# pkuyzy/ESC-GNN

Measured on AMD Instinct MI355X. Metric: graphs/sec + edges-aggregated/sec, NestedGIN_eff h=3 bs=128 @1/2/4/8 GPU, higher is better.
Workload: dtype f32; 1 GPU; count_cycle-shaped random regular graphs (n in 10/15/20/30), target=triangles, NestedGIN_eff h=3 layers=4 hidden=256, bs=128 per GPU (configs[1]); global_batch=128, parallelism=dp1 graph-sharded, rccl_ranks=1, ranks=1

## Files before the change

esc-gnn_amd/_native.py:

```python
import ctypes
import os
from ctypes import c_double, c_int64

from . import _abi

_HERE = os.path.dirname(os.path.abspath(__file__))
LIB_PATH = os.path.join(_HERE, "libescgnn_hip.so")


class NativeLibraryError(ImportError):
    pass


try:
    _ABI = _abi.load()
except OSError as exc:
    raise NativeLibraryError("esc_gnn_amd: cannot read the C header %s the binding is derived from (%s)" % (_abi.HEADER, exc)) from exc


def const(name):
    return _ABI.constants[name]


def struct(name):
# ... 45 lines not shown
LAPPE_SIGNATURES = {name: args for name, (args, _) in _LAPPE.functions.items()}
_RET.update({name: ret for name, (_, ret) in _LAPPE.functions.items()})
RWSE_HEADER = os.path.join(os.path.dirname(_abi.HEADER), "escgnn_rwse.h")
try:
    _RWSE = _abi.load(RWSE_HEADER)
except OSError as exc:
    raise NativeLibraryError("esc_gnn_amd: cannot read the C header %s the binding is derived from (%s)" % (RWSE_HEADER, exc)) from exc
RWSE_SIGNATURES = {name: args for name, (args, _) in _RWSE.functions.items()}
_RET.update({name: ret for name, (_, ret) in _RWSE.functions.items()})
STEP_HEADER = os.path.join(os.path.dirname(_abi.HEADER), "escgnn_step.h")
try:
    _STEP = _abi.load(STEP_HEADER)
except OSError as exc:
    raise NativeLibraryError("esc_gnn_amd: cannot read the C header %s the binding is derived from (%s)" % (STEP_HEADER, exc)) from exc
STEP_SIGNATURES = {name: args for name, (args, _) in _STEP.functions.items()}
_RET.update({name: ret for name, (_, ret) in _STEP.functions.items()})
GATEDGCN_HEADER = os.path.join(os.path.dirname(_abi.HEADER), "escgnn_gatedgcn.h")
try:
    _GATED = _abi.load(GATEDGCN_HEADER)
except OSError as exc:
    raise NativeLibraryError("esc_gnn_amd: cannot read the C header %s the binding is derived from (%s)" % (GATEDGCN_HEADER, exc)) from exc
GATEDGCN_SIGNATURES = {name: args for name, (args, _) in _GATED.functions.items()}
_RET.update({name: ret for name, (_, ret) in _GATED.functions.items()})
KIND = {name[len("ESC_K_"):].lower(): v for name, v in _ABI.enum.items() if name != "ESC_K_COUNT"}

CollateArgs = struct("esc_collate_args")
BnFuse = struct("esc_bn_fuse")
BnFold = struct("esc_bn_fold")
BnBwdFused = struct("esc_bn_bwd_fused")
BnBwdNext = struct("esc_bn_bwd_next")
SumJob = struct("esc_sum_job")
ReduceJob = struct("esc_reduce_job")

_lib = None


def lib():
    global _lib
    if _lib is not None:
        return _lib
    if not os.path.exists(LIB_PATH):
        raise NativeLibraryError(
            "esc_gnn_amd: %s not found. The HIP hot path has no fallback — build it with "
            "`python -c 'import __graft_entry__ as g; g.build()'` or `make -C esc-gnn_amd/csrc`." % LIB_PATH)
    h = ctypes.CDLL(LIB_PATH)
    for name, args in list(SIGNATURES.items()) + list(EXTENSION_SIGNATURES.items()) + list(I2GNN_SIGNATURES.items()) + list(GINEPLUS_SIGNATURES.items()) + list(GPS_SIGNATURES.items()) + list(LAPPE_SIGNATURES.items()) + list(RWSE_SIGNATURES.items()) + list(STEP_SIGNATURES.items()) + list(GATEDGCN_SIGNATURES.items()):
        try:
            fn = getattr(h, name)
        except AttributeError as exc:
            raise NativeLibraryError("esc_gnn_amd: %s lacks symbol %s (stale build?)" % (LIB_PATH, name)) from exc
        fn.argtypes = args
        fn.restype = _RET[name]
    if h.esc_abi_version() != ABI_VERSION:
        raise NativeLibraryError("esc_gnn_amd: ABI version mismatch (library %d, header %d) — rebuild"
                                 % (h.esc_abi_version(), ABI_VERSION))
    _lib = h
    return h


def call(name, *args):
    h = lib()
    rc = getattr(h, name)(*args)
    if rc != 0:
        raise RuntimeError("%s failed (%d): %s" % (name, rc, h.esc_last_error().decode()))


def ptr(t):
    return None if t is None else t.data_ptr()

# ... 35 lines not shown
```

esc-gnn_amd/csrc/engine.hip:

```cpp
#include "common.h"
#include "../../include/escgnn_step.h"

#include <map>
#include <vector>
#include <cstdlib>

namespace esc {

struct Arena {
  float* base;
  int64_t off;
  float* take(int64_t n) {
    float* p = base ? base + off : nullptr;
    off += (n + 63) & ~63LL;
    return p;
  }
};

struct BnWs { float *mean, *invstd, *scale, *shift, *nglob, *coef; };
struct MlpWs { float *Y0, *Y1; BnWs b0, b1; float* A1 = nullptr; };

struct Layout {
  int64_t N, E, Z, H, L, C0, W;
  float *Zb, *Yz; BnWs zb0, zb1;
// ... 117 lines not shown
  return esc_linear_bwd_both_deferred(dY, ld_dy, X, ld_x, sc, sh, lin.w, K, M, N, K, dX, ld_dx, accumulate, lin.dw, K, lin.db,
                                      slabs, &c.jobs->back(), c.s);
}

static constexpr bool kBnBwdApplyInGemm = true;
static constexpr bool kBnBwdSumsFromDx = true;
static constexpr bool kBnBwdSumsFromAgg = true;
static esc_bn_bwd_fused bn_fused(const float* x, int64_t ld_x, const BnWs& w, int relu) {
  return esc_bn_bwd_fused{x, ld_x, w.mean, w.invstd, w.scale, w.shift, w.coef, relu};
}
static int linear_backward_bn(const Ctx& c, const float* dOut, int64_t ld_dout, const esc_bn_bwd_fused& f, const float* X, int64_t ld_x,
                              const float* sc, const float* sh, const esc_linear_t& lin, int64_t M, float* dX, int64_t ld_dx,
                              int accumulate, const esc_bn_bwd_next* next) {
  const LdsFloorGuard cap(c.on_edge_stream);
  const int64_t N = lin.out_dim, K = lin.in_dim;
  if (c.jobs == nullptr)
    return esc_linear_bwd_both_bn(dOut, ld_dout, &f, X, ld_x, sc, sh, lin.w, K, M, N, K, dX, ld_dx, accumulate, lin.dw, K, lin.db, c.y.slabs,
                                  nullptr, next, c.s);
  float* slabs = *c.slab_cursor;
  *c.slab_cursor += (esc_linear_bwd_weight_scratch(M, N, K) + 63) & ~63LL;
  c.jobs->emplace_back();
  return esc_linear_bwd_both_bn(dOut, ld_dout, &f, X, ld_x, sc, sh, lin.w, K, M, N, K, dX, ld_dx, accumulate, lin.dw, K, lin.db, slabs,
                                &c.jobs->back(), next, c.s);
}

struct EdgeStream {
  hipStream_t stream = nullptr;
  hipEvent_t z_ready = nullptr, joined = nullptr, lin1_fork = nullptr, lin1_rest = nullptr, lin1_dw = nullptr, e_ready[ESC_MAX_LAYERS] = {}, de_ready[ESC_MAX_LAYERS] = {},
             agg_done[ESC_MAX_LAYERS] = {};
  hipEvent_t caller_done = nullptr, late_done = nullptr;
  bool ok = false;
};
static int g_use_edge_stream = 1;
static int current_device() {
  int dev = 0;
  (void)hipGetDevice(&dev);
  return dev;
}
static EdgeStream& edge_stream() {
  static thread_local std::map<int, EdgeStream> per_device;
  static thread_local EdgeStream off;
  if (!g_use_edge_stream) return off;
  EdgeStream& es = per_device[current_device()];
  if (!es.ok && es.stream == nullptr) {
    int least = 0, greatest = 0;
    (void)hipDeviceGetStreamPriorityRange(&least, &greatest);
// ... 192 lines not shown
}

struct MlpFuse { bool lin1 = false, lin0 = false; };
static MlpFuse mlp_fuse_plan(const Ctx& c, const esc_mlp_t& p, const MlpWs& w, const float* A, int64_t ld_a, int64_t M, const float* out,
                             int64_t ld_out, const float* dOut, int64_t ld_dout, const float* dA, int64_t ld_da, bool pre_out) {
  const Layout& y = c.y;
  const int64_t H = y.H;
  MlpFuse f;
  if (!(kBnBwdApplyInGemm && c.train && !sync_on(c) && y.bst_part != nullptr && p.lin1.in_dim == H && p.lin1.out_dim == H)) return f;
  if (!(c.act == 1 && w.A1 == nullptr)) return f;
  const esc_bn_bwd_fused f1 = bn_fused(pre_out ? out : w.Y1, pre_out ? ld_out : H, w.b1, c.act), f0 = bn_fused(w.Y0, H, w.b0, c.act);
  const esc_bn_bwd_next n0{y.bst_part, w.Y0, H, w.b0.mean, w.b0.invstd, w.b0.scale, w.b0.shift, c.act};
  const float* slab_probe = c.jobs ? *c.slab_cursor : y.slabs;
  f.lin1 = esc_linear_bwd_both_bn_ok(dOut, ld_dout, &f1, w.Y0, H, p.lin1.w, H, M, H, H, y.dT2, H, slab_probe, &n0) != 0;
  f.lin0 = f.lin1 && esc_linear_bwd_both_bn_ok(y.dT2, H, &f0, A, ld_a, p.lin0.w, p.lin0.in_dim, M, H, p.lin0.in_dim, dA, ld_da, slab_probe, nullptr) != 0;
  return f;
}
static bool mlp_backward_fused(const Ctx& c, const esc_mlp_t& p, const MlpWs& w, const float* A, int64_t ld_a, int64_t M, const float* out,
                               int64_t ld_out, const float* dOut, int64_t ld_dout, const float* dA, int64_t ld_da, bool pre_out) {
  return mlp_fuse_plan(c, p, w, A, ld_a, M, out, ld_out, dOut, ld_dout, dA, ld_da, pre_out).lin1;
}
static int mlp_backward(const Ctx& c, const esc_mlp_t& p, const MlpWs& w, const float* A, int64_t ld_a, int64_t M,
                        const float* out, int64_t ld_out, const float* dOut, int64_t ld_dout, float* dA,
                        int64_t ld_da, bool pre_out = false, int64_t have_slots = 0) {
  const Layout& y = c.y;
  const int64_t H = y.H;
  const MlpFuse fuse = mlp_fuse_plan(c, p, w, A, ld_a, M, out, ld_out, dOut, ld_dout, dA, ld_da, pre_out);
  if (fuse.lin1) {
    const float* x1 = pre_out ? out : w.Y1;
    const int64_t ld_x1 = pre_out ? ld_out : H;
    const esc_bn_bwd_fused f1 = bn_fused(x1, ld_x1, w.b1, c.act), f0 = bn_fused(w.Y0, H, w.b0, c.act);
    esc_bn_bwd_next n0{y.bst_part, w.Y0, H, w.b0.mean, w.b0.invstd, w.b0.scale, w.b0.shift, c.act};
    if (have_slots > 0)
      ESC_TRY(esc_bn_bwd_coef_from_partials(y.bst_part, have_slots, M, H, w.b1.coef, p.bn1.dgamma, p.bn1.dbeta, c.s));
    else
      ESC_TRY(esc_bn_bwd_coef(x1, ld_x1, nullptr, 0, dOut, ld_dout, M, H, w.b1.mean, w.b1.invstd, p.bn1.gamma, p.bn1.beta, c.act, w.b1.coef,
                              p.bn1.dgamma, p.bn1.dbeta, y.bn_scratch, c.s));
    ESC_TRY(linear_backward_bn(c, dOut, ld_dout, f1, w.Y0, H, w.b0.scale, w.b0.shift, p.lin1, M, y.dT2, H, 0, &n0));
    ESC_TRY(esc_bn_bwd_coef_from_partials(y.bst_part, cdiv(M, esc_linear_bwd_bn_block_rows(M, H, H)), M, H, w.b0.coef, p.bn0.dgamma, p.bn0.dbeta, c.s));
    if (fuse.lin0) return linear_backward_bn(c, y.dT2, H, f0, A, ld_a, nullptr, nullptr, p.lin0, M, dA, ld_da, 0, nullptr);
    ESC_TRY(esc_bn_bwd_apply(w.Y0, H, nullptr, 0, y.dT2, H, M, H, w.b0.mean, w.b0.invstd, p.bn0.gamma, p.bn0.beta, c.act, w.b0.coef, y.dT2, H, c.s));
    return linear_backward(c, y.dT2, H, A, ld_a, nullptr, nullptr, p.lin0, M, dA, ld_da, 0);
  }
  if (pre_out) ESC_TRY(bn_backward(c, out, ld_out, nullptr, 0, dOut, ld_dout, M, w.b1, p.bn1, y.dT1, H, y.bn_scratch));
  else         ESC_TRY(bn_backward(c, w.Y1, H, out, ld_out, dOut, ld_dout, M, w.b1, p.bn1, y.dT1, H, y.bn_scratch));
  if (w.A1) {
    ESC_TRY(linear_backward(c, y.dT1, H, w.A1, H, nullptr, nullptr, p.lin1, M, y.dT2, H, 0));
    ESC_TRY(bn_backward(c, w.Y0, H, w.A1, H, y.dT2, H, M, w.b0, p.bn0, y.dT2, H, y.bn_scratch));
    return linear_backward(c, y.dT2, H, A, ld_a, nullptr, nullptr, p.lin0, M, dA, ld_da, 0);
  }
  ESC_TRY(linear_backward(c, y.dT1, H, w.Y0, H, w.b0.scale, w.b0.shift, p.lin1, M, y.dT2, H, 0));
  ESC_TRY(bn_backward(c, w.Y0, H, nullptr, 0, y.dT2, H, M, w.b0, p.bn0, y.dT2, H, y.bn_scratch));
  return linear_backward(c, y.dT2, H, A, ld_a, nullptr, nullptr, p.lin0, M, dA, ld_da, 0);
}

static int forward(const Ctx& c) {
  const esc_nested_gin_t* m = c.m;
  const esc_batch_t* b = c.b;
  const Layout& y = c.y;
  const int64_t N = y.N, E = y.E, H = y.H, L = y.L, W = y.W;
  EdgeStream& es = edge_stream_for(E);
  Ctx ce = c;
// ... 198 lines not shown
    }
    if (!k0_split && hipEventRecord(es.lin1_rest, es.stream) != hipSuccess) { set_error("esc_engine: stream event failed"); return ESC_ELAUNCH; }
    const bool leave = fuse_l && fa_l && kBnBwdSumsFromDx && lin1_ok(K0, H, &nl) &&
                       mlp_backward_fused(c, m->conv[L - 1].nn, y.conv[L - 1], y.agg[L - 1], L == 1 ? y.C0 : H, N, y.cat + L * H, W, y.dcat + L * H, W,
                                          y.dagg, L == 1 ? y.C0 : H, true);
    ESC_TRY(part(c.s, K0, H, m->lin1.db, leave ? &nl : nullptr));
    if (leave) last_slots = cdiv(N, esc_linear_bwd_bn_block_rows(N, H, H));
  } else if (fuse_l) {
    ESC_TRY(linear_backward_bn(c, y.dAl, H, fl, y.cat, W, fa_l ? y.cat_scale : nullptr, fa_l ? y.cat_shift : nullptr, m->lin1, N, y.dcat, W, 0, nullptr));
  } else {
    ESC_TRY(linear_backward(c, y.dAl, H, y.cat, W, fa_l ? y.cat_scale : nullptr, fa_l ? y.cat_shift : nullptr, m->lin1, N, y.dcat, W, 0));
  }
  Ctx ce = es.ok ? edge_ctx(c, es.stream) : c;
  std::vector<esc_reduce_job> edge_jobs;
  edge_jobs.reserve(ESC_MAX_REDUCE_JOBS);
  if (es.ok && c.jobs) ce.jobs = &edge_jobs;
  std::vector<esc_sum_job> eps_jobs;
  int64_t agg_slots = 0;
  for (int l = (int)L - 1; l >= 0; --l) {
    const esc_conv_t& cv = m->conv[l];
    const int64_t C = l == 0 ? y.C0 : H;
    const float* hin = l == 0 ? b->x : y.cat + (int64_t)l * H;
    const int64_t ld_h = l == 0 ? y.C0 : W;
    ESC_TRY(mlp_backward(c, cv.nn, y.conv[l], y.agg[l], C, N, y.cat + (int64_t)(l + 1) * H, W,
                         y.dcat + (int64_t)(l + 1) * H, W, y.dagg, C, fuse_node_act(c), l == (int)L - 1 ? last_slots : agg_slots));
    agg_slots = 0;
    float* dx = l == 0 ? nullptr : y.dcat + (int64_t)l * H;
    if (split_lin1 && l == (int)L - 1 &&
        hipStreamWaitEvent((hipStream_t)c.s, es.lin1_rest, 0) != hipSuccess) { set_error("esc_engine: stream event failed"); return ESC_ELAUNCH; }
    const ArmedEvent arm(es.de_ready[l], es.ok);
    const bool stats_here = fuse_node_act(c) && l > 0 && kBnBwdSumsFromAgg && esc_gine_aggregate_bwd_deps_slots(C) == 1 && C <= 2048 &&
                            mlp_backward_fused(c, m->conv[l - 1].nn, y.conv[l - 1], y.agg[l - 1], l - 1 == 0 ? y.C0 : H, N, y.cat + (int64_t)l * H, W,
                                               y.dcat + (int64_t)l * H, W, y.dagg, l - 1 == 0 ? y.C0 : H, true);
    if (stats_here) {
      ESC_TRY(esc_gine_aggregate_bwd_affine_stats(hin, ld_h, y.cat_scale + (int64_t)l * H, y.cat_shift + (int64_t)l * H, y.conv[l - 1].b1.mean,
                                                  y.conv[l - 1].b1.invstd, y.e[l], y.ld_e[l], y.dagg, C, b->out_ptr, b->out_edge, b->out_dst, cv.eps, N, C,
                                                  y.d_e[l], C, dx, W, 1, y.deps_part + (int64_t)l * 2 * N, y.bst_part, c.s));
      agg_slots = esc_gine_aggregate_bwd_stats_slots(N);
    } else if (fuse_node_act(c) && l > 0)
      ESC_TRY(esc_gine_aggregate_bwd_affine(hin, ld_h, y.cat_scale + (int64_t)l * H, y.cat_shift + (int64_t)l * H, y.e[l], y.ld_e[l], y.dagg, C,
                                            b->out_ptr, b->out_edge, b->out_dst, cv.eps, N, C, y.d_e[l], C, dx, W, 1,
                                            y.deps_part + (int64_t)l * 2 * N, c.s));
    else
      ESC_TRY(esc_gine_aggregate_bwd(hin, ld_h, y.e[l], y.ld_e[l], y.dagg, C, b->out_ptr, b->out_edge, b->out_dst, cv.eps, N, C,
                                     y.d_e[l], C, dx, W, 1, y.deps_part + (int64_t)l * 2 * N, c.s));
    eps_jobs.push_back(esc_sum_job{y.deps_part + (int64_t)l * 2 * N, N * esc_gine_aggregate_bwd_deps_slots(C), cv.deps});
    if (es.ok) ESC_TRY(chain_armed(es.de_ready[l], arm, (hipStream_t)c.s, es.stream));
    const float* zin = y.Zemb;
    if (l == 0 && es.ok && c.jobs) {
      {
        const LdsFloorGuard cap(true);
        ESC_TRY(esc_linear_bwd_input(y.d_e[l], C, cv.lin.w, H, E, C, H, y.dZemb, H, l == (int)L - 1 ? 0 : 1, es.stream));
      }
      float* slabs = *c.slab_cursor;
      *c.slab_cursor += (esc_linear_bwd_weight_scratch(E, C, H) + 63) & ~63LL;
      c.jobs->emplace_back();
      ESC_TRY(esc_linear_bwd_both_deferred(y.d_e[l], C, zin, H, nullptr, nullptr, cv.lin.w, H, E, C, H, nullptr, 0, 0, cv.lin.dw, H, cv.lin.db,
                                           slabs, &c.jobs->back(), c.s));
    } else {
      ESC_TRY(linear_backward(ce, y.d_e[l], C, zin, H, nullptr, nullptr, cv.lin, E, y.dZemb, H, l == (int)L - 1 ? 0 : 1));
    }
    if (es.ok && !edge_jobs.empty() && l > 0) {
      ESC_TRY(esc_slab_reduce_jobs(edge_jobs.data(), (int)edge_jobs.size(), es.stream));
      edge_jobs.clear();
    }
  }
  ESC_TRY(mlp_backward(c, m->xemb, y.xemb, b->x, y.C0, N, y.cat, W, y.dcat, W, nullptr, 0, fuse_node_act(c)));
  Ctx ct = ce;
  ct.on_edge_stream = false;
  ESC_TRY(bn_backward(ce, y.Yz, H, nullptr, 0, y.dZemb, H, E, y.zb1, m->zbn1, y.dZemb, H, ce.y.bn_scratch));
  ESC_TRY(linear_backward(ct, y.dZemb, H, y.A0, H, nullptr, nullptr, m->zlin, E, y.dAz, H, 0));
  ESC_TRY(bn_backward(ce, y.Zb, H, nullptr, 0, y.dAz, H, E, y.zb0, m->zbn0, y.dAz, H, ce.y.bn_scratch));
  ESC_TRY(esc_bag_bwd_table_rows(y.dAz, H, H, b->col_ptr, b->col_row, b->col_val, b->col_col, y.Z, m->z_rows, E,
                                 1, m->dz_table, y.bag_scratch, ce.s));
  mark(PH_NODE_BWD_DONE, c.s);
  mark(PH_EDGE_BWD_DONE, ce.s);
  if (!eps_jobs.empty()) ESC_TRY(esc_reduce_sum_jobs(eps_jobs.data(), (int)eps_jobs.size(), c.s));
  if (k0_split && hipStreamWaitEvent((hipStream_t)c.s, es.lin1_dw, 0) != hipSuccess) { set_error("esc_engine: stream event failed"); return ESC_ELAUNCH; }
  if (c.jobs && !c.jobs->empty()) ESC_TRY(esc_slab_reduce_jobs(c.jobs->data(), (int)c.jobs->size(), c.s));
  if (es.ok) {
    if (!g_legacy_seam) {
      const ArmedEvent arm(es.joined, !edge_jobs.empty());
      if (!edge_jobs.empty()) ESC_TRY(esc_slab_reduce_jobs(edge_jobs.data(), (int)edge_jobs.size(), es.stream));
      edge_jobs.clear();
      ESC_TRY(chain_armed(es.joined, arm, es.stream, nullptr));
// ... 526 lines not shown

static void arm_jobs(Ctx& c, JobList& l, float* slabs, int64_t budget, bool always = false) {
  if (!always) l.jobs.reserve(ESC_MAX_REDUCE_JOBS);
  l.cursor = slabs;
  if (always || budget <= ESC_MAX_REDUCE_JOBS) { c.jobs = &l.jobs; c.slab_cursor = &l.cursor; }
}

}

using namespace esc;

extern "C" {

int esc_engine_set_two_stream_min_edges(int64_t edges) {
  g_two_stream_min_edges = edges < 0 ? 0 : edges;
  return ESC_OK;
}

int esc_engine_set_side_stream(int on) {
  g_use_edge_stream = (on & 2) != 0;
  g_plain_events = (on & 64) != 0;
  g_readout_one_launch = (on & 128) != 0;
  g_legacy_seam = (on & 256) != 0;
  seam_reset();
  return ESC_OK;
}

int esc_engine_adam_step(float* param, const float* grad, float* exp_avg, float* exp_avg_sq, int64_t n, int64_t n_early,
                         double lr, double beta1, double beta2, double eps, int64_t step, void* stream) {
  ESC_REQUIRE(param && grad && exp_avg && exp_avg_sq, "esc_engine_adam_step: null pointer");
  ESC_REQUIRE(n >= 0 && n_early >= 0 && n_early <= n && step >= 1, "esc_engine_adam_step: bad n/n_early/step");
  Seam& sm = seam();
  const bool split = sm.stage == 1 && !g_legacy_seam && sm.stream == (hipStream_t)stream && n_early < n &&
                     sm.z_table >= param + n_early && sm.z_table < param + n && sm.dz_table >= grad + n_early && sm.dz_table < grad + n;
  seam_reset();
  if (!split) return adam_launch(param, grad, exp_avg, exp_avg_sq, n, lr, beta1, beta2, eps, step, nullptr, stream);
  EdgeStream& es = edge_stream();
  if (!es.ok) return adam_launch(param, grad, exp_avg, exp_avg_sq, n, lr, beta1, beta2, eps, step, nullptr, stream);
  if (hipStreamWaitEvent(es.stream, es.caller_done, 0) != hipSuccess) { set_error("esc_engine: stream event failed"); return ESC_ELAUNCH; }
  {
    const ArmedEvent arm(es.late_done, true);
    ESC_TRY(adam_launch(param + n_early, grad + n_early, exp_avg + n_early, exp_avg_sq + n_early, n - n_early, lr, beta1, beta2, eps, step,
                        nullptr, es.stream));
    ESC_TRY(chain_armed(es.late_done, arm, es.stream, nullptr));
  }
  ESC_TRY(adam_launch(param, grad, exp_avg, exp_avg_sq, n_early, lr, beta1, beta2, eps, step, nullptr, stream));
// ... 261 lines not shown
```

esc-gnn_amd/csrc/linear_mfma.hip:

```cpp
#include "common.h"
#include <cstdlib>
#include "linear_plan.h"
#include "gemm_tile.h"
#include "gemm_dma.h"
#include "linear_small.h"
#include "linear_narrow.h"

namespace esc {

using plan::Flags;
using plan::Op;
using plan::Plan;

static plan::PlanKnobs g_plan;
void set_linear_knob(int knob, int value) {
  if (knob == 11) g_plan.use_dma = value;
  else if (knob == 14) g_plan.dual_split = value;
  else g_plan.knob[knob] = value;
}
static thread_local DualSplit t_dual_split;
static thread_local bool t_dual_split_on = false;
void request_dual_split(const DualSplit& r) { t_dual_split = r; t_dual_split_on = true; }
bool take_dual_split() { const bool pending = t_dual_split_on; t_dual_split_on = false; t_dual_split = DualSplit{}; return pending; }
static const plan::PlanKnobs& knobs() {
  static const bool env_read = [] {
    if (getenv("ESC_BIG_MIN_WGS")) g_plan.big_min_wgs = atoll(getenv("ESC_BIG_MIN_WGS"));
    if (getenv("ESC_TILE160")) g_plan.tile160 = atoi(getenv("ESC_TILE160"));
    if (getenv("ESC_TILE160_MIN_WGS")) g_plan.tile160_min_wgs = atoll(getenv("ESC_TILE160_MIN_WGS"));
    return true;
  }();
  (void)env_read;
  return g_plan;
}

using DmaBnCfg = dma::Cfg<64, 64, 32, 2, 2, 2, 2, false, true, 4, false, false>;
static_assert(DmaBnCfg::BNB_MAXK == BNB_MAX_N && DmaBnCfg::PRO_MAXK == PRO_MAX_K, "linear_plan.h and gemm_dma.h disagree on the LDS-resident vectors");
static_assert(plan::R01_TILE[1].bm == 64 && plan::R01_TILE[1].bn == 64 && plan::R01_TILE[1].bk == 32 && plan::R01_TILE[1].kw == 1, "tile 1 is the default tile");

static Flags pro_flags(const float* in_scale, const float* in_shift) {
// ... 95 lines not shown
  switch (p.family) {
    case plan::F_DMA64X32:
      return pro ? dma::launch_gemm<ESC_T64X32, false, false, 1, false, false>(g, 0, s)
                 : dma::launch_gemm<ESC_T64X32, false, false, 0, false, false>(g, 0, s);
    case plan::F_DMA160: return pro ? ESC_DMA_FWD(1, ESC_T160) : ESC_DMA_FWD(0, ESC_T160);
    case plan::F_DMA128: return pro ? ESC_DMA_FWD(1, ESC_T128) : ESC_DMA_FWD(0, ESC_T128);
    case plan::F_DMA128X64: return ESC_DMA_FWD(0, ESC_T128X64);
    default: return pro ? ESC_DMA_FWD(1, ESC_T64) : ESC_DMA_FWD(0, ESC_T64);
  }
#undef ESC_DMA_FWD
#undef ESC_DMA_FWD_FROM
}
static dma::GArgs dma_fwd_args(const float* X, int64_t ld_x, const float* W, int64_t ld_w, const float* bias, const float* in_scale,
                               const float* in_shift, int64_t M, int64_t N, int64_t K, float* Y, int64_t ld_y, float* col_stats) {
  dma::GArgs g{};
  g.A = X; g.lda = (int)ld_x; g.B = W; g.ldb = (int)ld_w; g.C = Y; g.ldc = (int)ld_y; g.bias = bias;
  g.pro_scale = in_scale; g.pro_shift = in_shift; g.col_stats = reinterpret_cast<float2*>(col_stats);
  g.M = (int)M; g.N = (int)N; g.R = (int)K; g.red_per_split = (int)K; g.accumulate = 0;
  return g;
}

static int launch_smalln_dx(const float* dY, int64_t ld_dy, const float* W, int64_t ld_w, int64_t M, int64_t N, int64_t K, float* dX,
                            int64_t ld_dx, int accumulate, const BnbDev& bd, int act, const char* what, hipStream_t s) {
  const size_t lds = (size_t)(32 + small::SMALL_MAX) * (N + 4) * sizeof(float);
  static size_t raised[3] = {64 * 1024, 64 * 1024, 64 * 1024};
  hipError_t e = hipSuccess;
  if (act == 0) e = dma::raise_lds(small::smalln_dx<small::SMALL_MAX>, lds, raised[0]);
  if (act != 0) e = dma::raise_lds(small::smalln_dx<small::SMALL_MAX, 1>, lds, raised[1]);
  if (e == hipSuccess && act == 2) e = dma::raise_lds(small::smalln_dx<small::SMALL_MAX, 2>, lds, raised[2]);
  if (dma_check(e, what) != hipSuccess) return ESC_ELAUNCH;
  auto kern = act == 0 ? small::smalln_dx<small::SMALL_MAX> : (act == 2 ? small::smalln_dx<small::SMALL_MAX, 2> : small::smalln_dx<small::SMALL_MAX, 1>);
  esc::launch(ESC_K_LINEAR, kern, dim3((unsigned)cdiv(M, 32)), dim3(256), lds, s, dY, ld_dy, W, ld_w, (int)M, (int)N, (int)K, dX, ld_dx, accumulate, bd);
  return ESC_OK;
}

static void launch_wgrad_small(const float* dY, int64_t ld_dy, const float* X, int64_t ld_x, const float* in_scale, const float* in_shift,
                               int64_t M, int64_t N, int64_t K, float* slabs, const Plan& p, const BnbDev& bd, int act, hipStream_t s) {
  float* db_part = slabs + (size_t)p.splits * N * K;
  const bool small_k = K <= small::SMALL_MAX;
  const dim3 grid((unsigned)p.splits, (unsigned)cdiv(small_k ? N : K, 256));
#define ESC_WGRAD_SMALL(...) \
  esc::launch(ESC_K_LINEAR, small::wgrad_small<small::SMALL_MAX, __VA_ARGS__>, grid, dim3(256), 0, s, dY, ld_dy, X, ld_x, in_scale, in_shift, (int)M, (int)N, (int)K, slabs, db_part, bd)
  if (act == 2)      { if (in_scale) ESC_WGRAD_SMALL(true, true, 2); else ESC_WGRAD_SMALL(true, false, 2); }
  else if (act == 1) { if (in_scale) ESC_WGRAD_SMALL(true, true, 1); else ESC_WGRAD_SMALL(true, false, 1); }
  else if (small_k)  { if (in_scale) ESC_WGRAD_SMALL(true, true); else ESC_WGRAD_SMALL(true, false); }
  else               { if (in_scale) ESC_WGRAD_SMALL(false, true); else ESC_WGRAD_SMALL(false, false); }
// ... 400 lines not shown
  dma_fill_dw(a.dw, dOut, ld_dout, X, ld_x, in_scale, in_shift, M, N, K, slabs, p);
  a.dx.bnb = bd; a.dw.bnb = bd;
  dma::DualEvents ev{};
  ev.split = p.launches == 2;
  ev.dx_lds = (size_t)p.dx_lds;
  if (ev.split && t_dual_split_on) { ev.dx_done = t_dual_split.dx_done; ev.dw_done = t_dual_split.dw_done; (void)take_dual_split(); }
  if (next)
    a.dx.bst = BnStatDev{reinterpret_cast<float2*>(next->partial), next->x, (int)next->ld_x, next->mean, next->invstd, next->scale, next->shift, next->relu};
  hipError_t e;
#define ESC_T64_2STAGE 64, 64, 32, 2, 2, 2, 2
  if (p.family == plan::F_DMA128_BN) {
    if (next) e = in_scale ? dma::launch_dual<ESC_T128, true, true, true>(a, 0, s, ESC_K_LINEAR, nullptr, ev) : dma::launch_dual<ESC_T128, false, true, true>(a, 0, s, ESC_K_LINEAR, nullptr, ev);
    else      e = in_scale ? dma::launch_dual<ESC_T128, true, true, false>(a, 0, s, ESC_K_LINEAR, nullptr, ev) : dma::launch_dual<ESC_T128, false, true, false>(a, 0, s, ESC_K_LINEAR, nullptr, ev);
  } else {
    if (bn == nullptr) e = in_scale ? dma::launch_dual<ESC_T64, true, false, true>(a, 0, s, ESC_K_LINEAR, nullptr, ev) : dma::launch_dual<ESC_T64, false, false, true>(a, 0, s, ESC_K_LINEAR, nullptr, ev);
    else if (next)     e = in_scale ? dma::launch_dual<ESC_T64_2STAGE, true, true, true>(a, 0, s, ESC_K_LINEAR, nullptr, ev) : dma::launch_dual<ESC_T64_2STAGE, false, true, true>(a, 0, s, ESC_K_LINEAR, nullptr, ev);
    else               e = in_scale ? dma::launch_dual<ESC_T64_2STAGE, true, true, false>(a, 0, s, ESC_K_LINEAR, nullptr, ev) : dma::launch_dual<ESC_T64_2STAGE, false, true, false>(a, 0, s, ESC_K_LINEAR, nullptr, ev);
  }
#undef ESC_T64_2STAGE
  if (dma_check(e, "esc_linear_bwd_both_bn") != hipSuccess) return ESC_ELAUNCH;
  return reduce_slabs(p, slabs, N, K, dW, ld_dw, db, defer, stream);
}

}
```

esc-gnn_amd/csrc/linear_small.h:

```cpp
#pragma once
#include "common.h"
#include "linear_plan.h"

namespace esc {
namespace small {


template <int KMAX>
__global__ __launch_bounds__(256) void smallk_fwd(const float* __restrict__ X, int64_t ldx, const float* __restrict__ W,
                                                  int64_t ldw, const float* __restrict__ bias, int M, int N, int K,
                                                  float* __restrict__ Y, int64_t ldy, float2* __restrict__ col_stats) {
  ESC_PRIO();
  __shared__ float xs[ROWS_FWD * KMAX];
  const int n = blockIdx.y * 256 + threadIdx.x;
  const int r0 = blockIdx.x * ROWS_FWD;
  const int rows = min(ROWS_FWD, M - r0);
  for (int i = threadIdx.x; i < ROWS_FWD * KMAX; i += 256) {
    const int r = i / KMAX, k = i % KMAX;
    xs[i] = (r < rows && k < K) ? X[(size_t)(r0 + r) * ldx + k] : 0.f;
  }
  float w[KMAX];
#pragma unroll
  for (int k = 0; k < KMAX; ++k) w[k] = (n < N && k < K) ? W[(size_t)n * ldw + k] : 0.f;
  const float b = (bias != nullptr && n < N) ? bias[n] : 0.f;
// ... 115 lines not shown
    *reinterpret_cast<float4*>(ys + r * ldn + c) = v;
  }
  for (int i = threadIdx.x; i < N * K; i += 256) wt[(i % K) * ldn + (i / K)] = W[(size_t)(i / K) * ldw + (i % K)];
  __syncthreads();
  const int r = threadIdx.x >> 3, ks = threadIdx.x & 7;
  if (r >= rows) return;
#pragma unroll
  for (int kk = 0; kk < KMAX / 8; ++kk) {
    const int k = ks + kk * 8;
    if (k >= K) break;
    float a0 = 0.f, a1 = 0.f, a2 = 0.f, a3 = 0.f;
    for (int c = 0; c < N; c += 4) {
      const float4 y = *reinterpret_cast<const float4*>(ys + r * ldn + c);
      const float4 w = *reinterpret_cast<const float4*>(wt + k * ldn + c);
      a0 = fmaf(y.x, w.x, a0); a1 = fmaf(y.y, w.y, a1); a2 = fmaf(y.z, w.z, a2); a3 = fmaf(y.w, w.w, a3);
    }
    float v = (a0 + a1) + (a2 + a3);
    float* dst = dX + (size_t)(r0 + r) * lddx + k;
    if (accumulate) v += *dst;
    *dst = v;
  }
}

}
}
```

esc-gnn_amd/csrc/runtime.hip:

```cpp
#include "common.h"
#include "linear_plan.h"
#include <algorithm>
#include <cstdlib>

#include <mutex>
#include <vector>

namespace esc {

static thread_local char g_err[512] = "";

void set_error(const char* fmt, ...) {
  va_list ap;
  va_start(ap, fmt);
  vsnprintf(g_err, sizeof(g_err), fmt, ap);
  va_end(ap);
}

struct ProfState {
  bool on = false;
  std::vector<hipEvent_t> start, stop;
  size_t used = 0;
};
static ProfState g_prof[ESC_K_COUNT];
// ... 80 lines not shown
  std::lock_guard<std::mutex> lk(g_ticket_mu);
  if (g_tickets[dev] == nullptr) {
    unsigned* p = nullptr;
    if (hipMalloc(&p, sizeof(unsigned) * TICKET_POOL) != hipSuccess) return nullptr;
    if (hipMemset(p, 0, sizeof(unsigned) * TICKET_POOL) != hipSuccess) { (void)hipFree(p); return nullptr; }
    g_tickets[dev] = p;
  }
  if (g_ticket_pos[dev] + n > TICKET_POOL) g_ticket_pos[dev] = 0;
  unsigned* out = g_tickets[dev] + g_ticket_pos[dev];
  g_ticket_pos[dev] += n;
  return out;
}

}

extern "C" {

int esc_tune_set(int knob, int value) {
  if (knob == 8) { esc::set_last_block_finalize(value); return ESC_OK; }
  if (knob == 9) { esc::set_norm_rowblock_cap(value); return ESC_OK; }
  if (knob == 12) { esc::set_bn_bwd_fold(value); return ESC_OK; }
  if (knob == 13) { esc::set_bn_bwd_one_launch(value); return ESC_OK; }
  if (knob == 10) { esc::set_edge_lds_floor(value); return ESC_OK; }
  ESC_REQUIRE(knob == 11 || knob == 14 || (knob >= 0 && knob < esc::plan::KNOB_COUNT), "esc_tune_set: unknown knob %d", knob);
  esc::set_linear_knob(knob, value);
  return ESC_OK;
}

int esc_abi_version(void) { return ESC_ABI_VERSION; }
const char* esc_last_error(void) { return esc::g_err; }

int esc_prof_enable(int kind, int on) {
  ESC_REQUIRE(kind >= 0 && kind < ESC_K_COUNT, "esc_prof_enable: bad kind %d", kind);
  std::lock_guard<std::mutex> lk(esc::g_prof_mu);
  esc::g_prof[kind].on = on != 0;
  return ESC_OK;
}

int esc_prof_reset(int kind) {
  ESC_REQUIRE(kind >= 0 && kind < ESC_K_COUNT, "esc_prof_reset: bad kind %d", kind);
  std::lock_guard<std::mutex> lk(esc::g_prof_mu);
  esc::g_prof[kind].used = 0;
  return ESC_OK;
}

int esc_prof_read(int kind, int64_t* launches, double* total_ms) {
  ESC_REQUIRE(kind >= 0 && kind < ESC_K_COUNT && launches && total_ms, "esc_prof_read: bad argument");
// ... 69 lines not shown
```

Before: 138,400 graphs/s.

## Split layer-0 lin0 backward into input and deferred weight halves; add lean small-N dX kernel

Result: no change. 138,100 graphs/s (-0.2%).

```diff
diff --git a/esc-gnn_amd/_native.py b/esc-gnn_amd/_native.py
--- a/esc-gnn_amd/_native.py
+++ b/esc-gnn_amd/_native.py
@@ -91,6 +91,13 @@
     raise NativeLibraryError("esc_gnn_amd: cannot read the C header %s the binding is derived from (%s)" % (GATEDGCN_HEADER, exc)) from exc
 GATEDGCN_SIGNATURES = {name: args for name, (args, _) in _GATED.functions.items()}
 _RET.update({name: ret for name, (_, ret) in _GATED.functions.items()})
+HANDOFF_HEADER = os.path.join(os.path.dirname(_abi.HEADER), "escgnn_handoff.h")
+try:
+    _HANDOFF = _abi.load(HANDOFF_HEADER)
+except OSError as exc:
+    raise NativeLibraryError("esc_gnn_amd: cannot read the C header %s the binding is derived from (%s)" % (HANDOFF_HEADER, exc)) from exc
+HANDOFF_SIGNATURES = {name: args for name, (args, _) in _HANDOFF.functions.items()}
+_RET.update({name: ret for name, (_, ret) in _HANDOFF.functions.items()})
 KIND = {name[len("ESC_K_"):].lower(): v for name, v in _ABI.enum.items() if name != "ESC_K_COUNT"}
 
 CollateArgs = struct("esc_collate_args")
@@ -113,7 +120,7 @@
             "esc_gnn_amd: %s not found. The HIP hot path has no fallback — build it with "
             "`python -c 'import __graft_entry__ as g; g.build()'` or `make -C esc-gnn_amd/csrc`." % LIB_PATH)
     h = ctypes.CDLL(LIB_PATH)
-    for name, args in list(SIGNATURES.items()) + list(EXTENSION_SIGNATURES.items()) + list(I2GNN_SIGNATURES.items()) + list(GINEPLUS_SIGNATURES.items()) + list(GPS_SIGNATURES.items()) + list(LAPPE_SIGNATURES.items()) + list(RWSE_SIGNATURES.items()) + list(STEP_SIGNATURES.items()) + list(GATEDGCN_SIGNATURES.items()):
+    for name, args in list(SIGNATURES.items()) + list(EXTENSION_SIGNATURES.items()) + list(I2GNN_SIGNATURES.items()) + list(GINEPLUS_SIGNATURES.items()) + list(GPS_SIGNATURES.items()) + list(LAPPE_SIGNATURES.items()) + list(RWSE_SIGNATURES.items()) + list(STEP_SIGNATURES.items()) + list(GATEDGCN_SIGNATURES.items()) + list(HANDOFF_SIGNATURES.items()):
         try:
             fn = getattr(h, name)
         except AttributeError as exc:
diff --git a/esc-gnn_amd/csrc/engine.hip b/esc-gnn_amd/csrc/engine.hip
--- a/esc-gnn_amd/csrc/engine.hip
+++ b/esc-gnn_amd/csrc/engine.hip
@@ -1,5 +1,6 @@
 #include "common.h"
 #include "../../include/escgnn_step.h"
+#include "../../include/escgnn_handoff.h"
 
 #include <map>
 #include <vector>
@@ -163,6 +164,42 @@
   c.jobs->emplace_back();
   return esc_linear_bwd_both_bn(dOut, ld_dout, &f, X, ld_x, sc, sh, lin.w, K, M, N, K, dX, ld_dx, accumulate, lin.dw, K, lin.db, slabs,
                                 &c.jobs->back(), next, c.s);
+}
+static int g_former_handoff = 0;
+struct HeldDw {
+  bool held = false;
+  const float* dOut = nullptr; int64_t ld_dout = 0;
+  esc_bn_bwd_fused f{};
+  const float* X = nullptr; int64_t ld_x = 0;
+  const esc_linear_t* lin = nullptr;
+  int64_t M = 0;
+  float* slabs = nullptr;
+  size_t job = 0;
+};
+static bool linear_backward_bn_halves(const Ctx& c, const float* dOut, int64_t ld_dout, const esc_bn_bwd_fused& f, const float* X, int64_t ld_x,
+                                      const esc_linear_t& lin, int64_t M, const float* dX, int64_t ld_dx) {
+  return !g_former_handoff && c.jobs != nullptr && dX != nullptr &&
+         esc_linear_bwd_bn_halves_ok(dOut, ld_dout, &f, X, ld_x, lin.w, lin.in_dim, M, lin.out_dim, lin.in_dim, dX, ld_dx, *c.slab_cursor) != 0;
+}
+static int linear_backward_bn_input(const Ctx& c, const float* dOut, int64_t ld_dout, const esc_bn_bwd_fused& f, const float* X, int64_t ld_x,
+                                    const esc_linear_t& lin, int64_t M, float* dX, int64_t ld_dx, int accumulate, HeldDw& h) {
+  const LdsFloorGuard cap(c.on_edge_stream);
+  const int64_t N = lin.out_dim, K = lin.in_dim;
+  h.dOut = dOut; h.ld_dout = ld_dout; h.f = f; h.X = X; h.ld_x = ld_x; h.lin = &lin; h.M = M;
+  h.slabs = *c.slab_cursor;
+  *c.slab_cursor += (esc_linear_bwd_weight_scratch(M, N, K) + 63) & ~63LL;
+  h.job = c.jobs->size();
+  c.jobs->emplace_back();
+  h.held = true;
+  return esc_linear_bwd_bn_input(dOut, ld_dout, &f, lin.w, K, M, N, K, dX, ld_dx, accumulate, c.s);
+}
+static int linear_backward_bn_weight(const Ctx& c, HeldDw& h) {
+  if (!h.held) return ESC_OK;
+  h.held = false;
+  const LdsFloorGuard cap(c.on_edge_stream);
+  const esc_linear_t& lin = *h.lin;
+  return esc_linear_bwd_bn_weight(h.dOut, h.ld_dout, &h.f, h.X, h.ld_x, nullptr, nullptr, h.M, lin.out_dim, lin.in_dim, lin.dw, lin.in_dim, lin.db,
+                                  h.slabs, &(*c.jobs)[h.job], c.s);
 }
 
 struct EdgeStream {
@@ -401,7 +438,7 @@
 }
 static int mlp_backward(const Ctx& c, const esc_mlp_t& p, const MlpWs& w, const float* A, int64_t ld_a, int64_t M,
                         const float* out, int64_t ld_out, const float* dOut, int64_t ld_dout, float* dA,
-                        int64_t ld_da, bool pre_out = false, int64_t have_slots = 0) {
+                        int64_t ld_da, bool pre_out = false, int64_t have_slots = 0, HeldDw* later = nullptr) {
   const Layout& y = c.y;
   const int64_t H = y.H;
   const MlpFuse fuse = mlp_fuse_plan(c, p, w, A, ld_a, M, out, ld_out, dOut, ld_dout, dA, ld_da, pre_out);
@@ -417,6 +454,8 @@
                               p.bn1.dgamma, p.bn1.dbeta, y.bn_scratch, c.s));
     ESC_TRY(linear_backward_bn(c, dOut, ld_dout, f1, w.Y0, H, w.b0.scale, w.b0.shift, p.lin1, M, y.dT2, H, 0, &n0));
     ESC_TRY(esc_bn_bwd_coef_from_partials(y.bst_part, cdiv(M, esc_linear_bwd_bn_block_rows(M, H, H)), M, H, w.b0.coef, p.bn0.dgamma, p.bn0.dbeta, c.s));
+    if (fuse.lin0 && later != nullptr && linear_backward_bn_halves(c, y.dT2, H, f0, A, ld_a, p.lin0, M, dA, ld_da))
+      return linear_backward_bn_input(c, y.dT2, H, f0, A, ld_a, p.lin0, M, dA, ld_da, 0, *later);
     if (fuse.lin0) return linear_backward_bn(c, y.dT2, H, f0, A, ld_a, nullptr, nullptr, p.lin0, M, dA, ld_da, 0, nullptr);
     ESC_TRY(esc_bn_bwd_apply(w.Y0, H, nullptr, 0, y.dT2, H, M, H, w.b0.mean, w.b0.invstd, p.bn0.gamma, p.bn0.beta, c.act, w.b0.coef, y.dT2, H, c.s));
     return linear_backward(c, y.dT2, H, A, ld_a, nullptr, nullptr, p.lin0, M, dA, ld_da, 0);
@@ -661,8 +700,10 @@
     const int64_t C = l == 0 ? y.C0 : H;
     const float* hin = l == 0 ? b->x : y.cat + (int64_t)l * H;
     const int64_t ld_h = l == 0 ? y.C0 : W;
+    HeldDw lin0_dw;
     ESC_TRY(mlp_backward(c, cv.nn, y.conv[l], y.agg[l], C, N, y.cat + (int64_t)(l + 1) * H, W,
-                         y.dcat + (int64_t)(l + 1) * H, W, y.dagg, C, fuse_node_act(c), l == (int)L - 1 ? last_slots : agg_slots));
+                         y.dcat + (int64_t)(l + 1) * H, W, y.dagg, C, fuse_node_act(c), l == (int)L - 1 ? last_slots : agg_slots,
+                         l == 0 ? &lin0_dw : nullptr));
     agg_slots = 0;
     float* dx = l == 0 ? nullptr : y.dcat + (int64_t)l * H;
     if (split_lin1 && l == (int)L - 1 &&
@@ -691,15 +732,17 @@
         const LdsFloorGuard cap(true);
         ESC_TRY(esc_linear_bwd_input(y.d_e[l], C, cv.lin.w, H, E, C, H, y.dZemb, H, l == (int)L - 1 ? 0 : 1, es.stream));
       }
+      ESC_TRY(linear_backward_bn_weight(c, lin0_dw));
       float* slabs = *c.slab_cursor;
       *c.slab_cursor += (esc_linear_bwd_weight_scratch(E, C, H) + 63) & ~63LL;
       c.jobs->emplace_back();
       ESC_TRY(esc_linear_bwd_both_deferred(y.d_e[l], C, zin, H, nullptr, nullptr, cv.lin.w, H, E, C, H, nullptr, 0, 0, cv.lin.dw, H, cv.lin.db,
                                            slabs, &c.jobs->back(), c.s));
     } else {
+      ESC_TRY(linear_backward_bn_weight(c, lin0_dw));
       ESC_TRY(linear_backward(ce, y.d_e[l], C, zin, H, nullptr, nullptr, cv.lin, E, y.dZemb, H, l == (int)L - 1 ? 0 : 1));
     }
-    if (es.ok && !edge_jobs.empty() && l > 0) {
+    if (es.ok && !edge_jobs.empty() && (l > 1 || (l == 1 && g_former_handoff))) {
       ESC_TRY(esc_slab_reduce_jobs(edge_jobs.data(), (int)edge_jobs.size(), es.stream));
       edge_jobs.clear();
     }
@@ -1272,6 +1315,7 @@
   g_plain_events = (on & 64) != 0;
   g_readout_one_launch = (on & 128) != 0;
   g_legacy_seam = (on & 256) != 0;
+  g_former_handoff = (on & 512) != 0;
   seam_reset();
   return ESC_OK;
 }
diff --git a/esc-gnn_amd/csrc/linear_mfma.hip b/esc-gnn_amd/csrc/linear_mfma.hip
--- a/esc-gnn_amd/csrc/linear_mfma.hip
+++ b/esc-gnn_amd/csrc/linear_mfma.hip
@@ -1,4 +1,5 @@
 #include "common.h"
+#include "../../include/escgnn_handoff.h"
 #include <cstdlib>
 #include "linear_plan.h"
 #include "gemm_tile.h"
@@ -13,8 +14,10 @@
 using plan::Plan;
 
 static plan::PlanKnobs g_plan;
+static int g_smalln_dx_32 = 0;
 void set_linear_knob(int knob, int value) {
-  if (knob == 11) g_plan.use_dma = value;
+  if (knob == 15) g_smalln_dx_32 = value != 0;
+  else if (knob == 11) g_plan.use_dma = value;
   else if (knob == 14) g_plan.dual_split = value;
   else g_plan.knob[knob] = value;
 }
@@ -156,6 +159,15 @@
 
 static int launch_smalln_dx(const float* dY, int64_t ld_dy, const float* W, int64_t ld_w, int64_t M, int64_t N, int64_t K, float* dX,
                             int64_t ld_dx, int accumulate, const BnbDev& bd, int act, const char* what, hipStream_t s) {
+  if (!g_smalln_dx_32) {
+    constexpr int R = small::SMALLN_LEAN_ROWS;
+    const size_t lds = (size_t)(R + small::SMALL_MAX) * (N + 4) * sizeof(float);
+    static size_t raised[3] = {64 * 1024, 64 * 1024, 64 * 1024};
+    auto kern = act == 0 ? small::smalln_dx_lean<small::SMALL_MAX> : (act == 2 ? small::smalln_dx_lean<small::SMALL_MAX, 2> : small::smalln_dx_lean<small::SMALL_MAX, 1>);
+    if (dma_check(dma::raise_lds(kern, lds, raised[act]), what) != hipSuccess) return ESC_ELAUNCH;
+    esc::launch(ESC_K_LINEAR, kern, dim3((unsigned)cdiv(M, R)), dim3(256), lds, s, dY, ld_dy, W, ld_w, (int)M, (int)N, (int)K, dX, ld_dx, accumulate, bd);
+    return ESC_OK;
+  }
   const size_t lds = (size_t)(32 + small::SMALL_MAX) * (N + 4) * sizeof(float);
   static size_t raised[3] = {64 * 1024, 64 * 1024, 64 * 1024};
   hipError_t e = hipSuccess;
@@ -602,4 +614,51 @@
   return reduce_slabs(p, slabs, N, K, dW, ld_dw, db, defer, stream);
 }
 
-}
+static Plan plan_bn_halves(const float* dOut, int64_t ld_dout, const esc_bn_bwd_fused* bn, const float* X, int64_t ld_x, const float* W,
+                           int64_t ld_w, int64_t M, int64_t N, int64_t K, const float* dX, int64_t ld_dx, const float* slabs) {
+  Plan none;
+  if (bn == nullptr) return none;
+  const Plan whole = plan_both_bn(dOut, ld_dout, bn, X, ld_x, W, ld_w, M, N, K, dX, ld_dx, slabs, nullptr);
+  return whole.ok && whole.family == plan::F_SMALL_BN ? whole : none;
+}
+static BnbDev bnb_dev(const esc_bn_bwd_fused* bn) {
+  return BnbDev{bn->x, (int)bn->ld_x, bn->mean, bn->invstd, bn->scale, bn->shift, reinterpret_cast<const float2*>(bn->coef), bn->relu};
+}
+
+int esc_linear_bwd_bn_halves_ok(const float* dOut, int64_t ld_dout, const void* bn_, const float* X, int64_t ld_x,
+                                const float* W, int64_t ld_w, int64_t M, int64_t N, int64_t K, const float* dX, int64_t ld_dx,
+                                const float* slabs) {
+  const esc_bn_bwd_fused* bn = static_cast<const esc_bn_bwd_fused*>(bn_);
+  return dX != nullptr && plan_bn_halves(dOut, ld_dout, bn, X, ld_x, W, ld_w, M, N, K, dX, ld_dx, slabs).ok ? 1 : 0;
+}
+
+int esc_linear_bwd_bn_input(const float* dOut, int64_t ld_dout, const void* bn_, const float* W, int64_t ld_w, int64_t M,
+                            int64_t N, int64_t K, float* dX, int64_t ld_dx, int accumulate, void* stream) {
+  const esc_bn_bwd_fused* bn = static_cast<const esc_bn_bwd_fused*>(bn_);
+  ESC_REQUIRE(dOut && bn && W && dX, "esc_linear_bwd_bn_input: null pointer");
+  const Plan p = plan_bn_halves(dOut, ld_dout, bn, W, ld_w, W, ld_w, M, N, K, dX, ld_dx, dOut);
+  ESC_REQUIRE(p.ok, "esc_linear_bwd_bn_input: shape / alignment not served (M=%ld N=%ld K=%ld) - use esc_linear_bwd_both_bn", (long)M, (long)N, (long)K);
+  const BnbDev bd = bnb_dev(bn);
+  ESC_TRY_(launch_smalln_dx(dOut, ld_dout, W, ld_w, M, N, K, dX, ld_dx, accumulate, bd, bd.relu == 2 ? 2 : 1, "esc_linear_bwd_bn_input",
+                            (hipStream_t)stream));
+  ESC_CHECK_LAUNCH("esc_linear_bwd_bn_input");
+  return ESC_OK;
+}
+
+int esc_linear_bwd_bn_weight(const float* dOut, int64_t ld_dout, const void* bn_, const float* X, int64_t ld_x,
+                             const float* in_scale, const float* in_shift, int64_t M, int64_t N, int64_t K, float* dW, int64_t ld_dw,
+                             float* db, float* slabs, void* job, void* stream) {
+  const esc_bn_bwd_fused* bn = static_cast<const esc_bn_bwd_fused*>(bn_);
+  esc_reduce_job* defer = static_cast<esc_reduce_job*>(job);
+  ESC_REQUIRE(dOut && bn && X && dW && slabs, "esc_linear_bwd_bn_weight: null pointer");
+  ESC_REQUIRE((in_scale == nullptr) == (in_shift == nullptr), "esc_linear_bwd_bn_weight: in_scale/in_shift must come together");
+  ESC_REQUIRE(ld_dw >= K, "esc_linear_bwd_bn_weight: bad sizes");
+  const Plan p = plan_bn_halves(dOut, ld_dout, bn, X, ld_x, X, ld_x, M, N, K, nullptr, 0, slabs);
+  ESC_REQUIRE(p.ok, "esc_linear_bwd_bn_weight: shape / alignment not served (M=%ld N=%ld K=%ld) - use esc_linear_bwd_both_bn", (long)M, (long)N, (long)K);
+  const BnbDev bd = bnb_dev(bn);
+  launch_wgrad_small(dOut, ld_dout, X, ld_x, in_scale, in_shift, M, N, K, slabs, p, bd, bd.relu == 2 ? 2 : 1, (hipStream_t)stream);
+  ESC_CHECK_LAUNCH("esc_linear_bwd_bn_weight");
+  return reduce_slabs(p, slabs, N, K, dW, ld_dw, db, defer, stream);
+}
+
+}
diff --git a/esc-gnn_amd/csrc/linear_small.h b/esc-gnn_amd/csrc/linear_small.h
--- a/esc-gnn_amd/csrc/linear_small.h
+++ b/esc-gnn_amd/csrc/linear_small.h
@@ -161,5 +161,91 @@
   }
 }
 
-}
-}
+constexpr int SMALLN_LEAN_ROWS = 16;
+struct Bnb4 { float4 mu, a, is, k01, k23, ms, mh; };
+__device__ __forceinline__ Bnb4 bnb_load4(const BnbDev& bnb, int c) {
+  Bnb4 k;
+  k.mu = *reinterpret_cast<const float4*>(bnb.mean + c); k.a = *reinterpret_cast<const float4*>(bnb.scale + c);
+  k.is = *reinterpret_cast<const float4*>(bnb.invstd + c);
+  k.k01 = *reinterpret_cast<const float4*>(bnb.coef + c); k.k23 = *reinterpret_cast<const float4*>(bnb.coef + c + 2);
+  k.ms = make_float4(0.f, 0.f, 0.f, 0.f); k.mh = make_float4(1.f, 1.f, 1.f, 1.f);
+  if (bnb.relu) { k.ms = k.a; k.mh = *reinterpret_cast<const float4*>(bnb.shift + c); }
+  return k;
+}
+template <int BNB>
+__device__ __forceinline__ float4 bnb_apply4(float4 v, const float4 x, const Bnb4& k) {
+  if constexpr (BNB == 2) {
+    v.x = bnb_apply_elu(v.x, x.x, k.mu.x, k.a.x, k.ms.x, k.mh.x, k.k01.x, k.is.x * k.k01.y); v.y = bnb_apply_elu(v.y, x.y, k.mu.y, k.a.y, k.ms.y, k.mh.y, k.k01.z, k.is.y * k.k01.w);
+    v.z = bnb_apply_elu(v.z, x.z, k.mu.z, k.a.z, k.ms.z, k.mh.z, k.k23.x, k.is.z * k.k23.y); v.w = bnb_apply_elu(v.w, x.w, k.mu.w, k.a.w, k.ms.w, k.mh.w, k.k23.z, k.is.w * k.k23.w);
+  } else {
+    v.x = bnb_apply(v.x, x.x, k.mu.x, k.a.x, k.ms.x, k.mh.x, k.k01.x, k.is.x * k.k01.y); v.y = bnb_apply(v.y, x.y, k.mu.y, k.a.y, k.ms.y, k.mh.y, k.k01.z, k.is.y * k.k01.w);
+    v.z = bnb_apply(v.z, x.z, k.mu.z, k.a.z, k.ms.z, k.mh.z, k.k23.x, k.is.z * k.k23.y); v.w = bnb_apply(v.w, x.w, k.mu.w, k.a.w, k.ms.w, k.mh.w, k.k23.z, k.is.w * k.k23.w);
+  }
+  return v;
+}
+template <int KMAX, int BNB = 0>
+__global__ __launch_bounds__(256) void smalln_dx_lean(const float* __restrict__ dY, int64_t lddy, const float* __restrict__ W,
+                                                      int64_t ldw, int M, int N, int K, float* __restrict__ dX, int64_t lddx,
+                                                      int accumulate, BnbDev bnb) {
+  static_assert(SMALLN_LEAN_ROWS * KMAX <= 256, "one (row, k) output per thread");
+  ESC_PRIO();
+  constexpr int WB = 8, YB = 2;
+  extern __shared__ __attribute__((aligned(16))) float sm[];
+  const int ldn = N + 4;
+  float* ys = sm;
+  float* wt = sm + SMALLN_LEAN_ROWS * ldn;
+  const int tid = threadIdx.x;
+  const int r0 = blockIdx.x * SMALLN_LEAN_ROWS;
+  const int rows = min(SMALLN_LEAN_ROWS, M - r0);
+  const int nk = N * K;
+  for (int base = tid; base < nk; base += WB * 256) {
+    float w[WB];
+    int at[WB];
+#pragma unroll
+    for (int j = 0; j < WB; ++j) {
+      const int i = min(base + j * 256, nk - 1), n = i / K, k = i - n * K;
+      at[j] = k * ldn + n;
+      w[j] = W[(size_t)n * ldw + k];
+    }
+#pragma unroll
+    for (int j = 0; j < WB; ++j)
+      if (base + j * 256 < nk) wt[at[j]] = w[j];
+  }
+  const int nq = N >> 2, items = rows * nq;
+  const bool fixed = 256 % nq == 0;
+  Bnb4 mine{};
+  if constexpr (BNB != 0) { if (fixed) mine = bnb_load4(bnb, (tid % nq) * 4); }
+  for (int base = tid; base < items; base += YB * 256) {
+    float4 v[YB], x[YB];
+    int r[YB], c[YB];
+#pragma unroll
+    for (int j = 0; j < YB; ++j) {
+      const int i = min(base + j * 256, items - 1);
+      r[j] = i / nq; c[j] = (i - r[j] * nq) * 4;
+      v[j] = *reinterpret_cast<const float4*>(dY + (size_t)(r0 + r[j]) * lddy + c[j]);
+      if constexpr (BNB != 0) x[j] = *reinterpret_cast<const float4*>(bnb.x + (size_t)(r0 + r[j]) * bnb.ldx + c[j]);
+    }
+#pragma unroll
+    for (int j = 0; j < YB; ++j) {
+      if (base + j * 256 >= items) break;
+      if constexpr (BNB != 0) v[j] = bnb_apply4<BNB>(v[j], x[j], fixed ? mine : bnb_load4(bnb, c[j]));
+      *reinterpret_cast<float4*>(ys + r[j] * ldn + c[j]) = v[j];
+    }
+  }
+  __syncthreads();
+  const int r = tid / K, k = tid - r * K;
+  if (r >= rows) return;
+  float a0 = 0.f, a1 = 0.f, a2 = 0.f, a3 = 0.f;
+  for (int c = 0; c < N; c += 4) {
+    const float4 y = *reinterpret_cast<const float4*>(ys + r * ldn + c);
+    const float4 w = *reinterpret_cast<const float4*>(wt + k * ldn + c);
+    a0 = fmaf(y.x, w.x, a0); a1 = fmaf(y.y, w.y, a1); a2 = fmaf(y.z, w.z, a2); a3 = fmaf(y.w, w.w, a3);
+  }
+  float v = (a0 + a1) + (a2 + a3);
+  float* dst = dX + (size_t)(r0 + r) * lddx + k;
+  if (accumulate) v += *dst;
+  *dst = v;
+}
+
+}
+}
diff --git a/esc-gnn_amd/csrc/runtime.hip b/esc-gnn_amd/csrc/runtime.hip
--- a/esc-gnn_amd/csrc/runtime.hip
+++ b/esc-gnn_amd/csrc/runtime.hip
@@ -126,7 +126,7 @@
   if (knob == 12) { esc::set_bn_bwd_fold(value); return ESC_OK; }
   if (knob == 13) { esc::set_bn_bwd_one_launch(value); return ESC_OK; }
   if (knob == 10) { esc::set_edge_lds_floor(value); return ESC_OK; }
-  ESC_REQUIRE(knob == 11 || knob == 14 || (knob >= 0 && knob < esc::plan::KNOB_COUNT), "esc_tune_set: unknown knob %d", knob);
+  ESC_REQUIRE(knob == 11 || knob == 14 || knob == 15 || (knob >= 0 && knob < esc::plan::KNOB_COUNT), "esc_tune_set: unknown knob %d", knob);
   esc::set_linear_knob(knob, value);
   return ESC_OK;
 }
diff --git a/include/escgnn_handoff.h b/include/escgnn_handoff.h
--- /dev/null
+++ b/include/escgnn_handoff.h
@@ -0,0 +1,21 @@
+#ifndef ESCGNN_HANDOFF_H
+#define ESCGNN_HANDOFF_H
+#include "escgnn_hip.h"
+
+#ifdef __cplusplus
+extern "C" {
+#endif
+
+int esc_linear_bwd_bn_halves_ok(const float* dOut, int64_t ld_dout, const void* bn, const float* X, int64_t ld_x,
+                                const float* W, int64_t ld_w, int64_t M, int64_t N, int64_t K, const float* dX, int64_t ld_dx,
+                                const float* slabs);
+int esc_linear_bwd_bn_input(const float* dOut, int64_t ld_dout, const void* bn, const float* W, int64_t ld_w, int64_t M,
+                            int64_t N, int64_t K, float* dX, int64_t ld_dx, int accumulate, void* stream);
+int esc_linear_bwd_bn_weight(const float* dOut, int64_t ld_dout, const void* bn, const float* X, int64_t ld_x,
+                             const float* in_scale, const float* in_shift, int64_t M, int64_t N, int64_t K, float* dW, int64_t ld_dw,
+                             float* db, float* slabs, void* job, void* stream);
+
+#ifdef __cplusplus
+}
+#endif
+#endif
```
